# DLR-RM/AugmentedAutoencoder

Hardware: AMD Instinct MI355X
Metric: crops/sec (encode+codebook-NN), 128x128x3 vs 92232x128 codebook, 1/8 GPU (higher is better)
Workload: dtype f32; 1 GPU; configs[1]: single object per GPU, batch=256 uint8 128x128x3 crops, HIP 4-conv encoder -> 128-d + cosine-NN vs 92232x128 fp32 codebook, top-1; batch_per_gpu=256, codebook_rows=92232, latent=128, parallelism=single GPU

## Files before the change

augmentedautoencoder_amd/csrc/kernels/conv_winograd_f32.h:

```cpp
#pragma once
#include <type_traits>

#include "multi_launch.h"

namespace aae {

struct ConvWinoArgs {
    const float* x;
    const float* U;
    const float* bias;
    const float* bn_scale;
    const float* bn_shift;
    float* out;
    int B, H, W, Cin, Cout, Ho, Wo;
    int eh, ew;
    int mode;
    int relu;
    int blocks_x, blocks_y;
    int regions;
    int xcd_cols;
#ifdef AAE_WINO_STAMPS
    long long* stamps;
#endif
};
#ifdef AAE_WINO_STAMPS
constexpr int kWinoStampSlots = 64;
#define AAE_WINO_STAMP(a, slot) do { if ((threadIdx.x & 63) == 0) (a).stamps[((size_t)blockIdx.x * 8 + (threadIdx.x >> 6)) * aae::kWinoStampSlots + (slot)] = aae::clock_ticks(); } while (0)
#else
#define AAE_WINO_STAMP(a, slot) do {} while (0)
#endif
inline unsigned wino_grid_blocks(int regions, int nbn, int xcd_cols) {
    if (xcd_cols <= 0) return (unsigned)regions * (unsigned)nbn;
    const int region_groups = 8 / (nbn / xcd_cols);
    return 8u * (unsigned)xcd_cols * (unsigned)((regions + region_groups - 1) / region_groups);
}
inline bool wino_xcd_cols_valid(int nbn, int xcd_cols) {
    return xcd_cols >= 1 && nbn % xcd_cols == 0 && (nbn / xcd_cols) <= 8 && 8 % (nbn / xcd_cols) == 0;
}

template <int GEOM>
struct WinoGeom;
template <>
struct WinoGeom<0> {
    static constexpr int kImages = 1, kRows = 18, kCols = 18, kRowPitch = 10, kParityPitch = 180, kImagePitch = 2 * 180, kPlane = 2 * 180 + 1;
    static constexpr int kFrameRows = 18, kFrameCols = 18;
    __host__ __device__ static constexpr int image_offset(int) { return 0; }
    __host__ __device__ static constexpr int frame_row(int) { return 0; }
    __host__ __device__ static constexpr int frame_col(int) { return 0; }
};
template <>
struct WinoGeom<1> {
    static constexpr int kImages = 4, kRows = 10, kCols = 10, kRowPitch = 10, kParityPitch = 190, kPlane = 2 * 190 + 1;
    static constexpr int kFrameRows = 19, kFrameCols = 20;
    __host__ __device__ static constexpr int image_offset(int i) { return 90 * (i >> 1) + 5 * (i & 1); }
    __host__ __device__ static constexpr int frame_row(int i) { return 9 * (i >> 1); }
    __host__ __device__ static constexpr int frame_col(int i) { return 10 * (i & 1); }
};
template <>
struct WinoGeom<2> {
    static constexpr int kImages = 4, kRows = 10, kCols = 10, kRowPitch = 6, kParityPitch = 60, kImagePitch = 128, kPlane = 4 * 128 + 1;
    static constexpr int kFrameRows = 10, kFrameCols = 10;
    __host__ __device__ static constexpr int image_offset(int i) { return i * kImagePitch; }
};
template <int GEOM>
constexpr int wino_plane_units() { return WinoGeom<GEOM>::kPlane; }
template <int GEOM>
constexpr int wino_stage_units() { return 8 * wino_plane_units<GEOM>(); }
template <int GEOM>
constexpr int wino_smem_bytes() { return 2 * wino_stage_units<GEOM>() * 16; }
template <int GEOM>
__host__ __device__ constexpr void wino_tile(int mh, int t, int& ti, int& ty, int& tx) {
    const int c = t >> 2, odd = (c ^ (c >> 1) ^ (c >> 2)) & 1;
    if (GEOM == 0) { ti = 0; ty = 4 * mh + (c >> 1); tx = 4 * odd + (t & 3); }
    else if (GEOM == 1) { ti = 2 * mh + odd; ty = c >> 1; tx = t & 3; }
    else { ti = 2 * mh + (t >> 4); ty = (t >> 2) & 3; tx = t & 3; }
}
template <int GEOM>
constexpr bool wino_geom_conflict_free() {
    using G = WinoGeom<GEOM>;
    for (int mh = 0; mh < 2; ++mh)
        for (int set = 0; set < 2; ++set) {
            unsigned seen = 0;
            for (int t = 0; t < 32; ++t) {
                const int c = t >> 2;
                if (((c ^ (c >> 1) ^ (c >> 2)) & 1) != set) continue;
                int ti = 0, ty = 0, tx = 0;
                wino_tile<GEOM>(mh, t, ti, ty, tx);
                seen |= 1u << ((G::image_offset(ti) + 2 * ty * G::kRowPitch + tx) & 15);
            }
            if (seen != 0xffffu) return false;
        }
    unsigned quads = 0;
    for (int cq = 0; cq < 8; ++cq) quads |= 1u << ((cq * G::kPlane) & 15);
    return __builtin_popcount(quads) == 8;
}
static_assert(wino_geom_conflict_free<0>() && wino_geom_conflict_free<1>(), "stage-buffer layouts: patch reads and fill stores free of bank conflicts");

struct ConvWinoLayerArgs {
    ConvWinoArgs c;
    const float* U4[4];
};
struct ConvWinoObject {
    const float* x;
    float* out;
    const float* U4[4];
    const float* bias;
    const float* bn_scale;
    const float* bn_shift;
    int B, pad_;
};
struct ConvWinoMultiArgs {
    ConvWinoArgs c;
    MultiRange range;
    ConvWinoObject obj[kMultiMax];
};
template <int GEOM, int STAGE_CH = 16>
constexpr int wino_layer_stage_bytes() { return 2 * (STAGE_CH / 4) * wino_plane_units<GEOM>() * 16; }
template <int GEOM, int STAGE_CH = 16>
constexpr int wino_layer_smem_bytes() { return wino_layer_stage_bytes<GEOM, STAGE_CH>() + 4 * 64 * 64 * 4; }
static_assert(wino_layer_smem_bytes<0, 32>() <= 160 * 1024 && wino_layer_smem_bytes<1, 32>() <= 160 * 1024 && wino_layer_smem_bytes<2, 16>() <= 160 * 1024, "LDS of a compute unit");
inline int wino_layer_geom_tag(int geom, bool static_halo) { return geom == 0 ? 0 : (static_halo ? 1 : 2); }
inline bool wino_layer_static_halo(int geom, int blocks_x, int blocks_y, bool option) { return option && (geom != 0 || (blocks_x == 1 && blocks_y == 1)); }
inline int wino_layer_stage_channels(int geom, int Cin, bool stage32, bool static_halo = true) {
    return stage32 && (geom == 0 || static_halo) && Cin % 32 == 0 ? 32 : 16;
}


#ifndef AAE_WINO_DECLARATIONS_ONLY

#if defined(__HIP_DEVICE_COMPILE__)
__device__ __forceinline__ f32x2 wino_pk_add(f32x2 a, f32x2 b) {
    f32x2 r;
    asm("v_pk_add_f32 %0, %1, %2" : "=v"(r) : "v"(a), "v"(b));
    return r;
}
__device__ __forceinline__ f32x2 wino_pk_sub(f32x2 a, f32x2 b) {
    f32x2 r;
    asm("v_pk_add_f32 %0, %1, %2 neg_lo:[0,1] neg_hi:[0,1]" : "=v"(r) : "v"(a), "v"(b));
    return r;
}
#else
__host__ __device__ inline f32x2 wino_pk_add(f32x2 a, f32x2 b) { return a + b; }
__host__ __device__ inline f32x2 wino_pk_sub(f32x2 a, f32x2 b) { return a - b; }
#endif
#if defined(__HIP_DEVICE_COMPILE__)
__device__ __forceinline__ f32x4 wino_fma4(float s, f32x4 a, f32x4 b) {
    const f32x2 ss = {s, s};
    f32x2 lo, hi;
    asm("v_pk_fma_f32 %0, %1, %2, %3" : "=v"(lo) : "v"(ss), "v"(a.lo), "v"(b.lo));
    asm("v_pk_fma_f32 %0, %1, %2, %3" : "=v"(hi) : "v"(ss), "v"(a.hi), "v"(b.hi));
    return f32x4{lo.x, lo.y, hi.x, hi.y};
}
#else
__host__ __device__ inline f32x4 wino_fma4(float s, f32x4 a, f32x4 b) {
    f32x4 r;
    for (int e = 0; e < 4; ++e) r[e] = fmaf(s, a[e], b[e]);
    return r;
}
#endif
__device__ __forceinline__ f32x4 wino_add4(f32x4 a, f32x4 b) {
    const f32x2 lo = wino_pk_add(a.lo, b.lo), hi = wino_pk_add(a.hi, b.hi);
    return f32x4{lo.x, lo.y, hi.x, hi.y};
}
__device__ __forceinline__ f32x4 wino_sub4(f32x4 a, f32x4 b) {
    const f32x2 lo = wino_pk_sub(a.lo, b.lo), hi = wino_pk_sub(a.hi, b.hi);
    return f32x4{lo.x, lo.y, hi.x, hi.y};
}
#if defined(__HIP_DEVICE_COMPILE__)
__device__ __forceinline__ float wino_add1(float a, float b) {
    float r;
    asm("v_add_f32 %0, %1, %2" : "=v"(r) : "v"(a), "v"(b));
    return r;
}
__device__ __forceinline__ float wino_sub1(float a, float b) {
    float r;
    asm("v_sub_f32 %0, %1, %2" : "=v"(r) : "v"(a), "v"(b));
    return r;
}
__device__ __forceinline__ float wino_nadd1(float a, float b) {
    float r;
    asm("v_sub_f32 %0, -%1, %2" : "=v"(r) : "v"(a), "v"(b));
    return r;
}
#else
__host__ __device__ inline float wino_add1(float a, float b) { return a + b; }
__host__ __device__ inline float wino_sub1(float a, float b) { return a - b; }
__host__ __device__ inline float wino_nadd1(float a, float b) { return -a - b; }
#endif
template <int N, int M>
__device__ __forceinline__ void wino_acc_fence(f32x16 (&c)[M]) {
#if defined(__HIP_DEVICE_COMPILE__)
    static_assert((N == 3 || N == 6 || N == 8) && N <= M, "PB or 2 PB accumulator tiles");
    if constexpr (N == 8)
        asm volatile("s_nop 15\n\ts_nop 3" : "+v"(c[0]), "+v"(c[1]), "+v"(c[2]), "+v"(c[3]), "+v"(c[4]), "+v"(c[5]), "+v"(c[6]), "+v"(c[7]));
    else if constexpr (N == 6)
        asm volatile("s_nop 15\n\ts_nop 3" : "+v"(c[0]), "+v"(c[1]), "+v"(c[2]), "+v"(c[3]), "+v"(c[4]), "+v"(c[5]));
    else
        asm volatile("s_nop 15\n\ts_nop 3" : "+v"(c[0]), "+v"(c[1]), "+v"(c[2]));
#else
    (void)c;
#endif
}

struct WinoBlock {
    int nb, region, img0, wy0, wx0;
    bool live;
};
__device__ __forceinline__ void wino_block_index(int block, int nbn, int regions, int xcd_cols, WinoBlock& w) {
    if (xcd_cols > 0) {
        const int col_groups = nbn / xcd_cols, region_groups = 8 / col_groups, chunk = (regions + region_groups - 1) / region_groups;
        const int xcd = block & 7, within = block >> 3, k = within / xcd_cols;
        w.nb = (xcd % col_groups) * xcd_cols + within % xcd_cols;
        w.region = (xcd / col_groups) * chunk + k;
        w.live = k < chunk && w.region < regions;
    } else {
        w.nb = block % nbn;
        w.region = block / nbn;
        w.live = w.region < regions;
    }
}
template <int GEOM>
__device__ __forceinline__ void wino_block_geometry(int local, int blocks_x, int blocks_y, WinoBlock& w) {
    if (GEOM == 0) {
        int rest = local;
        const int bx = rest % blocks_x;
        rest /= blocks_x;
        const int by = rest % blocks_y;
        w.img0 = rest / blocks_y;
        w.wy0 = 16 * by - 1;
        w.wx0 = 16 * bx - 1;
    } else {
        w.img0 = 4 * local;
        w.wy0 = w.wx0 = -1;
    }
}
template <int GEOM>
__device__ __forceinline__ WinoBlock wino_block(int block, int nbn, int blocks_x, int blocks_y, int regions, int xcd_cols) {
    WinoBlock w;
    wino_block_index(block, nbn, regions, xcd_cols, w);
    wino_block_geometry<GEOM>(w.region, blocks_x, blocks_y, w);
    return w;
}


template <int GEOM, int STAGE_CH, int NT, bool STATIC = false>
struct WinoFillPlan {
    using G = WinoGeom<GEOM>;
    static constexpr int kQuads = STAGE_CH / 4, kParts = STAGE_CH / 16;
    static constexpr int kDataRows = G::kRows - 2, kDataCols = G::kCols - 2;
    static constexpr int kStageQuads = G::kImages * (STATIC ? kDataRows * kDataCols : G::kRows * G::kCols) * kQuads;
    static constexpr int kPer = ((kStageQuads + NT - 1) / NT + kParts - 1) / kParts;
    static_assert(!STATIC || kStageQuads % (NT * kParts) == 0, "static halo: every thread has the same number of slots");
    static_assert(STATIC || GEOM != 1, "the mosaic's shared zero row needs the static halo");
    uint32_t goff[kParts * kPer];
    int lslot[kParts * kPer];
    __host__ __device__ static constexpr bool wave_stores(int wave, int i) { return STATIC || wave * 64 + NT * i < kStageQuads; }
    static constexpr int kSpareColumn = (G::kCols + 1) / 2;
    static_assert(STATIC || (kSpareColumn < G::kRowPitch && 64 / kQuads <= 2 * G::kRows), "spare units of the stage buffer");
    static_assert(NT % kQuads == 0, "a pixel's quads in one slot round");
    static constexpr int kHaloRows = G::kFrameRows - (G::kFrameRows / (kDataRows + 1)) * kDataRows;
    static constexpr int kHaloCols = G::kFrameCols - (G::kFrameCols / (kDataCols + 2)) * kDataCols;
    static constexpr int kHalo = kHaloRows * G::kFrameCols + (G::kFrameRows - kHaloRows) * kHaloCols;
    static_assert(!STATIC || kHalo + G::kImages * kDataRows * kDataCols == G::kFrameRows * G::kFrameCols, "halo + data = the frame");
};
constexpr uint32_t kWinoOutside = 0x80000000u;
template <int GEOM>
__host__ __device__ constexpr int wino_frame_unit(int fy, int fx) { return (fx & 1) * WinoGeom<GEOM>::kParityPitch + fy * WinoGeom<GEOM>::kRowPitch + (fx >> 1); }
template <int GEOM, int QUADS>
__host__ __device__ constexpr void wino_fill_pixel(int p, int& fy, int& fx) {
    using G = WinoGeom<GEOM>;
    constexpr int DR = G::kRows - 2, DC = G::kCols - 2;
    int wi = p / (DR * DC), dy = p % (DR * DC) / DC, dx = p % DC;
    if (QUADS == 4 && GEOM == 0) {
        const int q = p >> 1;
        wi = 0; dy = q / (DC / 2); dx = (q % (DC / 2)) + (p & 1) * (DC / 2);
    } else if (QUADS == 4) {
        const int q = p >> 1, r = q / DC;
        wi = r >> 2; dy = (r & 1) + 2 * (p & 1) + 4 * ((r >> 1) & 1); dx = q % DC;
    }
    fy = G::frame_row(wi) + 1 + dy;
    fx = G::frame_col(wi) + 1 + dx;
}
template <int GEOM, int QUADS>
constexpr bool wino_fill_order_valid() {
    using G = WinoGeom<GEOM>;
    constexpr int DR = G::kRows - 2, DC = G::kCols - 2, N = G::kImages * DR * DC;
    bool seen[G::kFrameRows * G::kFrameCols] = {};
    for (int p = 0; p < N; ++p) {
        int fy = 0, fx = 0;
        wino_fill_pixel<GEOM, QUADS>(p, fy, fx);
        if (seen[fy * G::kFrameCols + fx]) return false;
        seen[fy * G::kFrameCols + fx] = true;
    }
    for (int p = 0; p < N; p += 8 / QUADS) {
        unsigned banks = 0;
        for (int l = 0; l < 8; ++l) {
            int fy = 0, fx = 0;
            wino_fill_pixel<GEOM, QUADS>(p + l / QUADS, fy, fx);
            banks |= 1u << ((wino_frame_unit<GEOM>(fy, fx) + (l % QUADS) * G::kPlane) & 7);
        }
        if (banks != 0xffu) return false;
    }
    return true;
}
static_assert(wino_fill_order_valid<0, 8>() && wino_fill_order_valid<0, 4>() && wino_fill_order_valid<1, 8>() && wino_fill_order_valid<1, 4>(),
              "static-halo fill order: every data position once, store groups free of bank conflicts");

template <int GEOM, int STAGE_CH, int NT, bool STATIC>
__device__ __forceinline__ void wino_fill_plan(const ConvWinoArgs& a, const WinoBlock& wb, WinoFillPlan<GEOM, STAGE_CH, NT, STATIC>& f) {
    using G = WinoGeom<GEOM>;
    using F = WinoFillPlan<GEOM, STAGE_CH, NT, STATIC>;
    constexpr int kPlane = wino_plane_units<GEOM>();
    const int cq_per_pixel = a.Cin / 4;
    if constexpr (STATIC) {
        const int cq = (int)threadIdx.x % F::kQuads;
#pragma unroll
        for (int i = 0; i < F::kParts * F::kPer; ++i) {
            const int p = ((int)threadIdx.x + NT * i) / F::kQuads, wi = p / (F::kDataRows * F::kDataCols), b = wb.img0 + wi;
            int fy, fx;
            wino_fill_pixel<GEOM, F::kQuads>(p, fy, fx);
            const int uu = fy - G::frame_row(wi) - 1, vv = fx - G::frame_col(wi) - 1;
            f.goff[i] = b < a.B ? (uint32_t)(((((size_t)b * a.H + 2 * uu) * a.W + 2 * vv) * cq_per_pixel + cq) * 16) : kWinoOutside;
            f.lslot[i] = cq * kPlane + wino_frame_unit<GEOM>(fy, fx);
        }
    } else {
        constexpr int kStep = NT / F::kQuads, kWindow = G::kRows * G::kCols;
        constexpr int kStepI = kStep / kWindow, kStepY = kStep % kWindow / G::kCols, kStepX = kStep % G::kCols;
        const int pixel0 = (int)threadIdx.x / F::kQuads, cq = (int)threadIdx.x % F::kQuads;
        int wi = pixel0 / kWindow, wy = pixel0 % kWindow / G::kCols, wx = pixel0 % G::kCols;
#pragma unroll
        for (int i = 0; i < F::kParts * F::kPer; ++i) {
            const int idx = (int)threadIdx.x + NT * i;
            f.goff[i] = kWinoOutside;
            if (idx < F::kStageQuads) {
                const int uu = wb.wy0 + wy, vv = wb.wx0 + wx, b = wb.img0 + wi;
                if (uu >= 0 && uu < a.Ho && vv >= 0 && vv < a.Wo && b < a.B)
                    f.goff[i] = (uint32_t)(((((size_t)b * a.H + 2 * uu) * a.W + 2 * vv) * cq_per_pixel + cq) * 16);
                f.lslot[i] = cq * kPlane + wi * G::kImagePitch + (wx & 1) * G::kParityPitch + wy * G::kRowPitch + (wx >> 1);
            } else {
                const int d = (idx - F::kStageQuads) & 63, row = d / F::kQuads;
                f.lslot[i] = cq * kPlane + (row / G::kRows) * G::kParityPitch + (row % G::kRows) * G::kRowPitch + F::kSpareColumn;
            }
            wx += kStepX;
            wy += kStepY + (wx >= G::kCols ? 1 : 0);
            wx -= wx >= G::kCols ? G::kCols : 0;
            wi += kStepI + (wy >= G::kRows ? 1 : 0);
            wy -= wy >= G::kRows ? G::kRows : 0;
        }
    }
}
template <int GEOM, int STAGE_CH, int NT>
__device__ __forceinline__ void wino_zero_halo(f32x4* lds) {
    using G = WinoGeom<GEOM>;
    using F = WinoFillPlan<GEOM, STAGE_CH, NT, true>;
    constexpr int kStage = F::kQuads * wino_plane_units<GEOM>(), kTotal = 2 * F::kQuads * F::kHalo;
    constexpr int kRowPart = F::kHaloRows * G::kFrameCols, kRowStep = (G::kFrameRows - 1) / (F::kHaloRows - 1);
#pragma unroll
    for (int i = 0; i < (kTotal + NT - 1) / NT; ++i) {
        const int idx = (int)threadIdx.x + NT * i;
        if (idx < kTotal) {
            const int hq = idx % (F::kQuads * F::kHalo), buf = idx / (F::kQuads * F::kHalo), cq = hq % F::kQuads, hp = hq / F::kQuads;
            int fy, fx;
            if (hp < kRowPart) {
                fy = (hp / G::kFrameCols) * kRowStep;
                fx = hp % G::kFrameCols;
            } else {
                const int k = hp - kRowPart, r = k / F::kHaloCols, c = k % F::kHaloCols;
                fy = 1 + r + r / F::kDataRows;
                fx = (c >> 1) * (F::kDataCols + 2) + (c & 1) * (F::kDataCols + 1);
            }
            lds[buf * kStage + cq * wino_plane_units<GEOM>() + wino_frame_unit<GEOM>(fy, fx)] = f32x4{0.f, 0.f, 0.f, 0.f};
        }
    }
}

template <int TA, int TB>
__device__ __forceinline__ void wino_first_fragments(const ConvWinoArgs& a, const float* U, const WinoBlock& wb, f32x4 (&u)[8]) {
    constexpr int PB = TB + 1, NP = (TA + 1) * PB;
    const int tid = threadIdx.x, lane = tid & 63, wave = wave_uniform(tid >> 6);
    const int nh = (wave >> 1) & 1, ph = wave >> 2, m = lane & 31, h = lane >> 5, n32 = wb.nb * 2 + nh, KG = a.Cin / 8;
    const buffer_rsrc urs = make_buffer(U, (uint32_t)((size_t)NP * a.Cin * a.Cout * 4));
    const uint32_t ulane = (uint32_t)(((size_t)n32 * KG * NP + (size_t)ph * 2 * PB) * 64 + h * 32 + m) * 16u;
    const bool two_rows = TA == 3 || ph == 0;
#pragma unroll
    for (int p = 0; p < 2 * PB; ++p) u[p] = buffer_load4_s(urs, ulane + (p % PB) * 1024u, two_rows ? (p / PB) * PB * 1024u : (p / PB) * (NP * 1024u));
}
template <int GEOM, int STAGE_CH, int NT, bool STATIC>
__device__ __forceinline__ void wino_first_stage(const ConvWinoArgs& a, int eh, int ew, const WinoFillPlan<GEOM, STAGE_CH, NT, STATIC>& fill, f32x4* lds) {
    using F = WinoFillPlan<GEOM, STAGE_CH, NT, STATIC>;
    const int wave = wave_uniform((int)threadIdx.x >> 6);
    const buffer_rsrc xrs = make_buffer(a.x, (uint32_t)((size_t)a.B * a.H * a.W * a.Cin * 4));
    const uint32_t parity_off = (uint32_t)(((size_t)eh * a.W + ew) * a.Cin * 4);
    f32x4 stg[F::kParts * F::kPer];
#pragma unroll
    for (int i = 0; i < F::kParts * F::kPer; ++i) stg[i] = buffer_load4_s(xrs, fill.goff[i], parity_off);
    if constexpr (STATIC) wino_zero_halo<GEOM, STAGE_CH, NT>(lds);
#pragma unroll
    for (int i = 0; i < F::kParts * F::kPer; ++i)
        if (F::wave_stores(wave, i)) lds[fill.lslot[i]] = stg[i];
    __syncthreads();
}

template <int TA, int TB, bool SWAP, int GEOM, int STAGE_CH, bool ACCUMULATE, bool WIDE, int CHAIN = 0, int NTA = 3, int NTB = 3, bool STATIC = false>
__device__ __forceinline__ void wino_phase_body(const ConvWinoArgs& a, const float* U, int eh, int ew, const WinoBlock& wb, f32x4* lds, float* xch_all,
                                                const WinoFillPlan<GEOM, STAGE_CH, WIDE ? 256 : 512, STATIC>& fill, int& buf0, f32x4 (&uin)[8],
                                                const float* Un, int neh, int new_, f32x4 (&uout)[8]) {
    using G = WinoGeom<GEOM>;
    using F = WinoFillPlan<GEOM, STAGE_CH, WIDE ? 256 : 512, STATIC>;
    constexpr int PB = TB + 1;
    constexpr int kQuads = STAGE_CH / 4, kGroups = STAGE_CH / 8;
    constexpr int kPlane = wino_plane_units<GEOM>(), kStage = kQuads * kPlane;
    constexpr int kParity = G::kParityPitch;
    constexpr int kParts = F::kParts, kPer = F::kPer;
    constexpr int NH = WIDE ? 2 : 1;
    constexpr int kOffA = TA == 2 ? 1 : 0, kOffB = TB == 2 ? 1 : 0;
    static_assert(!STATIC || (CHAIN & 1), "the static halo is written in front of the chained form's first stage (wino_first_stage)");
    static_assert(CHAIN == 0 || !WIDE, "the chained form passes one wave's weight fragments between the components");
    const int tid = threadIdx.x, lane = tid & 63, wave = wave_uniform(tid >> 6);
    const int mh = wave & 1, nh = WIDE ? 0 : (wave >> 1) & 1, ph = WIDE ? wave >> 1 : wave >> 2, m = lane & 31, h = lane >> 5;
    int li, lty, ltx;
    wino_tile<GEOM>(mh, m, li, lty, ltx);
    const int n32 = wb.nb * 2 + nh, KG = a.Cin / 8, nst = a.Cin / STAGE_CH;
    constexpr int NP = (TA + 1) * PB;
    constexpr int kPhaseNo = TA == 3 && TB == 3 ? 0 : (TA == 3 && !SWAP ? 1 : (TA == 3 ? 2 : 3));
    (void)kPhaseNo;
    AAE_WINO_STAMP(a, 4 * kPhaseNo + 0);
    const buffer_rsrc xrs = make_buffer(a.x, (uint32_t)((size_t)a.B * a.H * a.W * a.Cin * 4));
    const buffer_rsrc urs = make_buffer(U, (uint32_t)((size_t)NP * a.Cin * a.Cout * 4));
    const uint32_t ulane = (uint32_t)(((size_t)n32 * KG * NP + (size_t)ph * 2 * PB) * 64 + h * 32 + m) * 16u;
    const bool two_rows = TA == 3 || ph == 0;
    const uint32_t parity_off = (uint32_t)(((size_t)eh * a.W + ew) * a.Cin * 4);
    const uint32_t next_parity_off = (uint32_t)(((size_t)neh * a.W + new_) * a.Cin * 4);

    f32x16 acc[NH][2 * PB];

    f32x4 stg[kPer];
    auto stage_load = [&](uint32_t soff, int part) {
#pragma unroll
        for (int i = 0; i < kPer; ++i) stg[i] = buffer_load4_s(xrs, fill.goff[part * kPer + i], soff);
    };
    auto stage_store = [&](int buf, int part) {
#pragma unroll
        for (int i = 0; i < kPer; ++i)
            if (F::wave_stores(wave, part * kPer + i)) lds[buf * kStage + fill.lslot[part * kPer + i]] = stg[i];
    };
    auto fA = [](int pos) { return SWAP ? (pos & 1) * kParity + (pos >> 1) : pos * G::kRowPitch; };
    auto fB = [](int pos) { return SWAP ? pos * G::kRowPitch : (pos & 1) * kParity + (pos >> 1); };
    const int lane_base = G::image_offset(li) + 2 * lty * G::kRowPitch + ltx;
    const int posA0 = (TA == 3 ? (ph == 0 ? 0 : 2) : (ph == 0 ? 0 : 1)) + kOffA;
    const int posA1 = (ph == 0 ? 1 : 3) + kOffA;
    const int posA2 = (TA == 3 ? (ph == 0 ? 2 : 1) : (ph == 0 ? 1 : 2)) + kOffA;
    const int offA0 = fA(posA0), offA1 = fA(posA1), offA2 = fA(posA2);
    const float sg = ph == 0 ? 1.f : -1.f;

    const uint32_t half_stride = (uint32_t)KG * NP * 1024u;
    f32x4 u[NH][2 * PB];
    if (CHAIN & 1) {
#pragma unroll
        for (int p = 0; p < 2 * PB; ++p) u[0][p] = uin[p];
    } else {
#pragma unroll
        for (int n2 = 0; n2 < NH; ++n2)
#pragma unroll
            for (int p = 0; p < 2 * PB; ++p)
                u[n2][p] = buffer_load4_s(urs, ulane + (p % PB) * 1024u, (two_rows ? (p / PB) * PB * 1024u : (p / PB) * (NP * 1024u)) + n2 * half_stride);
#pragma unroll
        for (int part = 0; part < kParts; ++part) {
            stage_load(parity_off, part);
            stage_store(buf0, part);
        }
        __syncthreads();
    }
    AAE_WINO_STAMP(a, 4 * kPhaseNo + 1);

    auto read_unit = [&](const f32x4* plane, int i, f32x4 (&raw)[2 * PB]) {
#pragma unroll
        for (int s2 = 0; s2 < PB; ++s2) {
            const int ob = fB(s2 + kOffB);
            if (i == 0) raw[s2] = plane[offA0 + ob];
            else if (TA == 3) raw[s2] = plane[offA1 + ob];
            if (i == 0) raw[PB + s2] = plane[offA2 + ob];
        }
    };
    auto step_a = [&](int i, const f32x4 (&raw)[2 * PB], f32x4 (&w)[PB]) {
#pragma unroll
        for (int s2 = 0; s2 < PB; ++s2) {
            if (i == 0) w[s2] = wino_sub4(raw[s2], raw[PB + s2]);
            else if (TA == 3) w[s2] = wino_fma4(sg, raw[s2], raw[PB + s2]);
            else w[s2] = raw[PB + s2];
        }
    };
    auto step_b = [&](f32x4 (&w)[PB]) {
        if (TB == 3) {
            const f32x4 e0 = w[0], e1 = w[1], e2 = w[2], e3 = w[PB - 1];
            w[0] = wino_sub4(e0, e2);
            w[1] = wino_add4(e1, e2);
            w[2] = wino_sub4(e2, e1);
            w[PB - 1] = wino_sub4(e1, e3);
        } else {
            const f32x4 e0 = w[0], e1 = w[1], e2 = w[2];
            w[0] = wino_sub4(e0, e1);
            w[2] = wino_sub4(e1, e2);
        }
    };
    auto run = [&](auto rows_tag) {
        constexpr int ROWS = decltype(rows_tag)::value, NU = kGroups * ROWS, kPartUnits = NU / kParts;
        static_assert(NU % 2 == 0 && NU % kParts == 0, "units per stage");
        constexpr int kStoreBack = kPartUnits >= 4 ? 2 : 1;
        const bool early = ph == 1 && kStoreBack == 2;
        f32x4 raw[2 * PB], v[PB];
        read_unit(lds + buf0 * kStage + h * kPlane + lane_base, 0, raw);
        auto stage_body = [&](int st, auto first_tag) {
            constexpr bool FIRST = decltype(first_tag)::value;
            const int buf = (buf0 + st) & 1;
            const bool more = st + 1 < nst;
            const bool filling = more || (CHAIN & 2);
            const uint32_t fill_off = more ? parity_off + (uint32_t)(st + 1) * kQuads * 16 : next_parity_off;
#ifdef AAE_WINO_STAMPS
            if (kPhaseNo == 0 && st < 8) AAE_WINO_STAMP(a, 20 + st);
#endif
            const f32x4* stage = lds + buf * kStage + h * kPlane + lane_base;
            const f32x4* next_stage = lds + (buf ^ 1) * kStage + h * kPlane + lane_base;
#pragma unroll
            for (int t = 0; t < NU; ++t) {
                const int i = t % ROWS, slot = t & 1;
#ifdef AAE_WINO_STAMPS
                if (kPhaseNo == 0 && (st == 2 || st == 3) && t < 4) AAE_WINO_STAMP(a, 28 + 6 * (st - 2) + t);
#endif
                step_a(i, raw, v);
                step_b(v);
                if ((!FIRST || t > 0) && (more || t + 1 < NU)) {
                    const int tn = (t + 1) % NU, gn = (st + (t + 1) / NU) * kGroups + tn / ROWS;
                    const uint32_t un = (uint32_t)gn * (NP * 1024u) + (tn % ROWS) * PB * 1024u;
#pragma unroll
                    for (int n2 = 0; n2 < NH; ++n2)
#pragma unroll
                        for (int j = 0; j < PB; ++j) u[n2][(slot ^ 1) * PB + j] = buffer_load4_s(urs, ulane + j * 1024u, un + n2 * half_stride);
                }
                if (filling && t % kPartUnits == 0) stage_load(fill_off, t / kPartUnits);
                if (filling && t % kPartUnits == kPartUnits - kStoreBack) stage_store(buf ^ 1, t / kPartUnits);
                if (t + 1 < NU) read_unit(stage + 2 * ((t + 1) / ROWS) * kPlane, (t + 1) % ROWS, raw);
                if (filling && (t == NU - 1 ? !early : (t == NU - 2 && early))) {
#ifdef AAE_WINO_STAMPS
                    if (kPhaseNo == 0 && (st == 2 || st == 3)) AAE_WINO_STAMP(a, 28 + 6 * (st - 2) + 4);
#endif
                    __syncthreads();
#ifdef AAE_WINO_STAMPS
                    if (kPhaseNo == 0 && (st == 2 || st == 3)) AAE_WINO_STAMP(a, 28 + 6 * (st - 2) + 5);
#endif
                }
                if (t == NU - 1 && more) read_unit(next_stage, 0, raw);
                sched_fence();
#pragma unroll
                for (int q = 0; q < 4; ++q)
#pragma unroll
                    for (int j = 0; j < PB; ++j)
#pragma unroll
                        for (int n2 = 0; n2 < NH; ++n2) {
                            f32x16& c = acc[n2][(ROWS == 2 ? i * PB : 0) + j];
                            if (FIRST && t < ROWS && q == 0) c = mfma_32x32x2(v[j][q], u[n2][slot * PB + j][q], f32x16{});
                            else c = mfma_32x32x2(v[j][q], u[n2][slot * PB + j][q], c);
                        }
                sched_fence();
            }
        };
        stage_body(0, std::true_type());
        for (int st = 1; st < nst; ++st) stage_body(st, std::false_type());
    };
    if (TA == 3 || ph == 0) run(std::integral_constant<int, 2>());
    else run(std::integral_constant<int, 1>());
    if (STAGE_CH == 32 && CHAIN == 0) __syncthreads();
    AAE_WINO_STAMP(a, 4 * kPhaseNo + 2);
    if (CHAIN & 2) {
        wino_first_fragments<NTA, NTB>(a, Un, wb, uout);
    }
    buf0 = (buf0 + nst) & 1;
#pragma unroll
    for (int n2 = 0; n2 < NH; ++n2) {
        if constexpr (TA == 2) {
            if (ph == 1) wino_acc_fence<PB>(acc[n2]);
            else wino_acc_fence<2 * PB>(acc[n2]);
        } else {
            wino_acc_fence<2 * PB>(acc[n2]);
        }
    }

    auto drain = [&](auto ph_tag) {
        constexpr int PH = decltype(ph_tag)::value;
        auto partial = [&](int n2, int r, float (&y)[4]) {
            constexpr bool kNoQ0 = PH == 1 && TA == 2;
            float q0[PB], q1[PB];
#pragma unroll
            for (int j = 0; j < PB; ++j) {
                const float mA = acc[n2][j][r], mB = kNoQ0 ? 0.f : acc[n2][PB + j][r];
                if (PH == 0) { q0[j] = wino_add1(mA, mB); q1[j] = mB; }
                else if (TA == 3) { q0[j] = mA; q1[j] = wino_nadd1(mA, mB); }
                else { q0[j] = 0.f; q1[j] = -mA; }
            }
            float t[4];
            if (TB == 3) {
                t[0] = kNoQ0 ? 0.f : wino_add1(wino_add1(q0[0], q0[1]), q0[2]);
                t[1] = kNoQ0 ? 0.f : wino_sub1(wino_sub1(q0[1], q0[2]), q0[3]);
                t[2] = wino_add1(wino_add1(q1[0], q1[1]), q1[2]);
                t[3] = wino_sub1(wino_sub1(q1[1], q1[2]), q1[3]);
            } else {
                t[0] = kNoQ0 ? 0.f : wino_add1(q0[0], q0[1]);
                t[1] = kNoQ0 ? 0.f : wino_sub1(q0[1], q0[2]);
                t[2] = wino_add1(q1[0], q1[1]);
                t[3] = wino_sub1(q1[1], q1[2]);
            }
            y[0] = t[0];
            y[1] = SWAP ? t[2] : t[1];
            y[2] = SWAP ? t[1] : t[2];
            y[3] = t[3];
        };
        f32x4 yv[NH][16];
#pragma unroll
        for (int n2 = 0; n2 < NH; ++n2)
#pragma unroll
            for (int r = 0; r < 16; ++r) {
                float y[4];
                partial(n2, r, y);
                yv[n2][r] = f32x4{y[0], y[1], y[2], y[3]};
            }
#ifdef AAE_WINO_STAMPS
        AAE_WINO_STAMP(a, 48 + 4 * kPhaseNo + 0);
#endif
#pragma unroll
        for (int round = 0; round < 2; ++round) {
            const int par = PH == round ? 0 : 1;
#pragma unroll
            for (int n2 = 0; n2 < NH; ++n2) {
                f32x4* xq = reinterpret_cast<f32x4*>(xch_all) + (size_t)(mh + 2 * (nh + n2)) * 16 * 64 + lane;
                if (ACCUMULATE || round == 1) {
                    f32x4 old[8];
#pragma unroll
                    for (int e = 0; e < 8; ++e) old[e] = xq[(2 * e + par) * 64];
#pragma unroll
                    for (int e = 0; e < 8; ++e) xq[(2 * e + par) * 64] = old[e] + yv[n2][2 * e + par];
                } else {
#pragma unroll
                    for (int e = 0; e < 8; ++e) xq[(2 * e + par) * 64] = yv[n2][2 * e + par];
                }
            }
#ifdef AAE_WINO_STAMPS
            asm volatile("s_waitcnt lgkmcnt(0)" ::: "memory");
            AAE_WINO_STAMP(a, 48 + 4 * kPhaseNo + 1 + 2 * round);
#endif
            if (round == 0 || !(CHAIN & 2) || nst < 2) __syncthreads();
#ifdef AAE_WINO_STAMPS
            if (round == 0) AAE_WINO_STAMP(a, 48 + 4 * kPhaseNo + 2);
#endif
        }
    };
    if (ph == 0) drain(std::integral_constant<int, 0>());
    else drain(std::integral_constant<int, 1>());
    AAE_WINO_STAMP(a, 4 * kPhaseNo + 3);
}

template <int GEOM, int NT>
__device__ __forceinline__ void wino_store_block(const ConvWinoArgs& a, int mode, const WinoBlock& wb, const float* xall) {
    const int tid = threadIdx.x;
    const int n4 = wb.nb * 64 + (tid & 15) * 4;
    f32x4 bs = {0.f, 0.f, 0.f, 0.f}, sc = {1.f, 1.f, 1.f, 1.f}, sh = {0.f, 0.f, 0.f, 0.f};
    if (mode >= 2) {
        bs = *reinterpret_cast<const f32x4*>(a.bias + n4);
        if (a.bn_scale) {
            sc = *reinterpret_cast<const f32x4*>(a.bn_scale + n4);
            sh = *reinterpret_cast<const f32x4*>(a.bn_shift + n4);
        }
    }
#pragma unroll
    for (int round = 0; round < 1024 / NT; ++round) {
        const int idx = tid + NT * round, cq = idx & 15, t = idx >> 4;
        const int tmh = t >> 5, mt = t & 31, tnh = cq >> 3;
        const int r = (mt & 3) + 4 * (mt >> 3), hh = (mt >> 2) & 1;
        const f32x4* src = reinterpret_cast<const f32x4*>(xall) + (size_t)(tmh + 2 * tnh) * 16 * 64 + r * 64 + 32 * hh + (cq & 7) * 4;
        const f32x4 c0 = src[0], c1 = src[1], c2 = src[2], c3 = src[3];
        int ti, ty, tx;
        wino_tile<GEOM>(tmh, mt, ti, ty, tx);
        const int b = wb.img0 + ti;
        if (b >= a.B) continue;
        const int oy = (GEOM == 0 ? wb.wy0 + 1 : 0) + 2 * ty, ox = (GEOM == 0 ? wb.wx0 + 1 : 0) + 2 * tx;
        float* o = a.out + (((size_t)b * a.Ho + oy) * a.Wo + ox) * a.Cout + wb.nb * 64 + cq * 4;
        float* optr[4] = {o, o + a.Cout, o + (size_t)a.Wo * a.Cout, o + (size_t)a.Wo * a.Cout + a.Cout};
        f32x4 val[4];
#pragma unroll
        for (int k = 0; k < 4; ++k) val[k] = f32x4{c0[k], c1[k], c2[k], c3[k]};
        if (mode == 1 || mode == 2) {
#pragma unroll
            for (int k = 0; k < 4; ++k) val[k] += *reinterpret_cast<const f32x4*>(optr[k]);
        }
        if (mode >= 2) {
#pragma unroll
            for (int k = 0; k < 4; ++k) {
                val[k] += bs;
                if (a.relu) {
#pragma unroll
                    for (int e = 0; e < 4; ++e) val[k][e] = fmaxf(val[k][e], 0.f);
                }
                if (a.bn_scale) val[k] = val[k] * sc + sh;
            }
        }
#pragma unroll
        for (int k = 0; k < 4; ++k) *reinterpret_cast<f32x4*>(optr[k]) = val[k];
    }
}

#ifdef AAE_EXPERIMENTS
template <int TA, int TB, bool SWAP, int GEOM>
__global__ __launch_bounds__(512) void conv_wino_phase_kernel(ConvWinoArgs a) {
    AAE_DYN_SMEM(smem_raw);
    const WinoBlock wb = wino_block<GEOM>(blockIdx.x, a.Cout / 64, a.blocks_x, a.blocks_y, a.regions, a.xcd_cols);
    if (!wb.live) return;
    WinoFillPlan<GEOM, 32, 512> fill;
    wino_fill_plan(a, wb, fill);
    int buf0 = 0;
    f32x4 unused[8];
    wino_phase_body<TA, TB, SWAP, GEOM, 32, false, false>(a, a.U, a.eh, a.ew, wb, reinterpret_cast<f32x4*>(smem_raw), reinterpret_cast<float*>(smem_raw), fill, buf0, unused,
                                                          nullptr, 0, 0, unused);
    wino_store_block<GEOM, 512>(a, a.mode, wb, reinterpret_cast<const float*>(smem_raw));
}
#endif

template <int GEOM, bool WIDE, int STAGE_CH, bool STATIC>
__device__ __forceinline__ void wino_layer_block(const ConvWinoArgs& a, const float* const (&U4)[4], const WinoBlock& wb, unsigned char* smem_raw) {
    constexpr int SC = STAGE_CH;
    static_assert(SC == 16 || (SC == 32 && !WIDE), "stage size");
    static_assert(!STATIC || !WIDE, "the static halo belongs to the chained form");
    f32x4* lds = reinterpret_cast<f32x4*>(smem_raw);
    float* xch = reinterpret_cast<float*>(smem_raw + wino_layer_stage_bytes<GEOM, SC>());
    WinoFillPlan<GEOM, SC, WIDE ? 256 : 512, STATIC> fill;
    int buf0 = 0;
    f32x4 ua[8], ub[8];
    if (!WIDE) wino_first_fragments<3, 3>(a, U4[3], wb, ua);
    wino_fill_plan(a, wb, fill);
    if constexpr (WIDE) {
        wino_phase_body<3, 3, false, GEOM, SC, false, WIDE>(a, U4[3], 1, 1, wb, lds, xch, fill, buf0, ua, nullptr, 0, 0, ub);
        wino_phase_body<3, 2, false, GEOM, SC, true, WIDE>(a, U4[2], 1, 0, wb, lds, xch, fill, buf0, ua, nullptr, 0, 0, ub);
        wino_phase_body<3, 2, true, GEOM, SC, true, WIDE>(a, U4[1], 0, 1, wb, lds, xch, fill, buf0, ua, nullptr, 0, 0, ub);
        wino_phase_body<2, 2, false, GEOM, SC, true, WIDE>(a, U4[0], 0, 0, wb, lds, xch, fill, buf0, ua, nullptr, 0, 0, ub);
    } else {
        constexpr bool W = WIDE;
        if (!W) wino_first_stage(a, 1, 1, fill, lds);
        wino_phase_body<3, 3, false, GEOM, SC, false, W, W ? 0 : 3, 3, 2, STATIC>(a, U4[3], 1, 1, wb, lds, xch, fill, buf0, ua, U4[2], 1, 0, ub);
        wino_phase_body<3, 2, false, GEOM, SC, true, W, W ? 0 : 3, 3, 2, STATIC>(a, U4[2], 1, 0, wb, lds, xch, fill, buf0, ub, U4[1], 0, 1, ua);
        wino_phase_body<3, 2, true, GEOM, SC, true, W, W ? 0 : 3, 2, 2, STATIC>(a, U4[1], 0, 1, wb, lds, xch, fill, buf0, ua, U4[0], 0, 0, ub);
        wino_phase_body<2, 2, false, GEOM, SC, true, W, W ? 0 : 1, 3, 3, STATIC>(a, U4[0], 0, 0, wb, lds, xch, fill, buf0, ub, nullptr, 0, 0, ua);
    }
    wino_store_block<GEOM, WIDE ? 256 : 512>(a, 3, wb, xch);
}

template <int GEOM, bool WIDE, int STAGE_CH = 16, bool STATIC = false>
__global__ __launch_bounds__(WIDE ? 256 : 512) void conv_wino_layer_kernel(ConvWinoLayerArgs p) {
    AAE_DYN_SMEM(smem_raw);
    const ConvWinoArgs& a = p.c;
    const WinoBlock wb = wino_block<GEOM>(blockIdx.x, a.Cout / 64, a.blocks_x, a.blocks_y, a.regions, a.xcd_cols);
    if (!wb.live) return;
    wino_layer_block<GEOM, WIDE, STAGE_CH, STATIC>(a, p.U4, wb, smem_raw);
#ifdef AAE_WINO_STAMPS
    asm volatile("s_waitcnt vmcnt(0)" ::: "memory");
    AAE_WINO_STAMP(a, 16);
    if (threadIdx.x == 0) a.stamps[((size_t)blockIdx.x * 8) * kWinoStampSlots + 17] = (long long)(__builtin_amdgcn_s_getreg(20 | (0 << 6) | (3 << 11)) & 15);
#endif
}

template <int GEOM, int STAGE_CH = 16, bool STATIC = false>
__global__ __launch_bounds__(512) void conv_wino_layer_multi_kernel(ConvWinoMultiArgs p) {
    AAE_DYN_SMEM(smem_raw);
    WinoBlock wb;
    wino_block_index(blockIdx.x, p.c.Cout / 64, p.c.regions, p.c.xcd_cols, wb);
    if (!wb.live) return;
    const int o = multi_find(p.range, wb.region);
    wino_block_geometry<GEOM>(wb.region - p.range.first[o], p.c.blocks_x, p.c.blocks_y, wb);
    ConvWinoArgs a = p.c;
    const ConvWinoObject& ob = p.obj[o];
    a.x = ob.x; a.out = ob.out; a.bias = ob.bias; a.bn_scale = ob.bn_scale; a.bn_shift = ob.bn_shift; a.B = ob.B;
    const float* U4[4] = {ob.U4[0], ob.U4[1], ob.U4[2], ob.U4[3]};
    wino_layer_block<GEOM, false, STAGE_CH, STATIC>(a, U4, wb, smem_raw);
}

#endif

}
```

Measured before the change: 58170 crops/s.

## Split static-halo fill across four waves and drain Winograd outputs in pairs

For the chained 32-channel static-halo Winograd layer, the input staging fill is handed to the four ph==0 waves, each holding one base offset plus compile-time strides, in place of per-slot offset tables spread over all eight waves. The output drain is reworked to pack element pairs with packed-float adds and write the exchange buffer as float4 pairs, with a matching pair-aware store routine and a permuted row-to-tile mapping. The aim is to cut fill-plan register use, the number of LDS transactions and the scalar drain instructions. In exchange, half the waves sit idle during fills, so the remaining waves carry a heavier load and more latency lands on the critical path.

Result: no change. 58070 crops/s (-0.2%).

```diff
diff --git a/augmentedautoencoder_amd/csrc/kernels/conv_winograd_f32.h b/augmentedautoencoder_amd/csrc/kernels/conv_winograd_f32.h
--- a/augmentedautoencoder_amd/csrc/kernels/conv_winograd_f32.h
+++ b/augmentedautoencoder_amd/csrc/kernels/conv_winograd_f32.h
@@ -75,6 +75,17 @@
     else if (GEOM == 1) { ti = 2 * mh + odd; ty = c >> 1; tx = t & 3; }
     else { ti = 2 * mh + (t >> 4); ty = (t >> 2) & 3; tx = t & 3; }
 }
+template <int STAGE_CH, bool WIDE>
+constexpr bool wino_drain_pairs() {
+#ifdef AAE_WINO_SCALAR_DRAIN
+    return false;
+#else
+    return STAGE_CH == 32 && !WIDE;
+#endif
+}
+template <bool PAIRS>
+__host__ __device__ constexpr int wino_row_tile(int m) { return PAIRS ? (m & ~3) | ((m & 1) << 1) | ((m >> 1) & 1) : m; }
+
 template <int GEOM>
 constexpr bool wino_geom_conflict_free() {
     using G = WinoGeom<GEOM>;
@@ -139,9 +150,15 @@
     asm("v_pk_add_f32 %0, %1, %2 neg_lo:[0,1] neg_hi:[0,1]" : "=v"(r) : "v"(a), "v"(b));
     return r;
 }
+__device__ __forceinline__ f32x2 wino_pk_nadd(f32x2 a, f32x2 b) {
+    f32x2 r;
+    asm("v_pk_add_f32 %0, %1, %2 neg_lo:[1,1] neg_hi:[1,1]" : "=v"(r) : "v"(a), "v"(b));
+    return r;
+}
 #else
 __host__ __device__ inline f32x2 wino_pk_add(f32x2 a, f32x2 b) { return a + b; }
 __host__ __device__ inline f32x2 wino_pk_sub(f32x2 a, f32x2 b) { return a - b; }
+__host__ __device__ inline f32x2 wino_pk_nadd(f32x2 a, f32x2 b) { return -a - b; }
 #endif
 #if defined(__HIP_DEVICE_COMPILE__)
 __device__ __forceinline__ f32x4 wino_fma4(float s, f32x4 a, f32x4 b) {
@@ -306,6 +323,84 @@
 static_assert(wino_fill_order_valid<0, 8>() && wino_fill_order_valid<0, 4>() && wino_fill_order_valid<1, 8>() && wino_fill_order_valid<1, 4>(),
               "static-halo fill order: every data position once, store groups free of bank conflicts");
 
+template <int GEOM, int STAGE_CH, bool WIDE, bool STATIC>
+constexpr bool wino_fill_split() {
+#ifdef AAE_WINO_FILL_ALL_WAVES
+    return false;
+#else
+    return STATIC && STAGE_CH == 32 && !WIDE;
+#endif
+}
+template <int GEOM>
+struct WinoFillSplit {
+    using G = WinoGeom<GEOM>;
+    using P = WinoFillPlan<GEOM, 32, 256, true>;
+    static constexpr int kQuads = P::kQuads, kParts = P::kParts, kPer = P::kPer, kSlots = kParts * kPer, kPixelStep = 256 / kQuads;
+    static_assert(kPer * 4 <= 16, "at most 16 staging registers live at a time");
+    uint32_t goff;
+    int lslot;
+    int images;
+    struct Step { int wi, uu, vv, units; };
+    __host__ __device__ static constexpr Step step_from(int p0, int i) {
+        constexpr int kImagePixels = P::kDataRows * P::kDataCols;
+        const int p = p0 + kPixelStep * i, wi0 = p0 / kImagePixels, wi = p / kImagePixels;
+        int fy0 = 0, fx0 = 0, fy = 0, fx = 0;
+        wino_fill_pixel<GEOM, kQuads>(p0, fy0, fx0);
+        wino_fill_pixel<GEOM, kQuads>(p, fy, fx);
+        return Step{wi - wi0, (fy - G::frame_row(wi)) - (fy0 - G::frame_row(wi0)), (fx - G::frame_col(wi)) - (fx0 - G::frame_col(wi0)),
+                    wino_frame_unit<GEOM>(fy, fx) - wino_frame_unit<GEOM>(fy0, fx0)};
+    }
+    __host__ __device__ static constexpr Step step(int i) { return step_from(0, i); }
+    static constexpr bool regular() {
+        for (int p0 = 0; p0 < kPixelStep; ++p0) {
+            if (p0 >= P::kDataRows * P::kDataCols) return false;
+            for (int i = 0; i < kSlots; ++i) {
+                const Step s = step_from(p0, i), s0 = step(i);
+                if (s.wi != s0.wi || s.uu != s0.uu || s.vv != s0.vv || s.units != s0.units) return false;
+            }
+        }
+        return true;
+    }
+    __host__ __device__ static uint32_t source_step(const ConvWinoArgs& a, int i) {
+        const Step s = step(i);
+        return (uint32_t)(((s.wi * a.H + 2 * s.uu) * a.W + 2 * s.vv) * a.Cin * 4);
+    }
+};
+static_assert(WinoFillSplit<0>::regular() && WinoFillSplit<1>::regular(), "the four-wave fill of the static halo: one offset pair per thread");
+template <int GEOM, int STAGE_CH, bool WIDE, bool STATIC>
+using WinoLayerFill = std::conditional_t<wino_fill_split<GEOM, STAGE_CH, WIDE, STATIC>(), WinoFillSplit<GEOM>, WinoFillPlan<GEOM, STAGE_CH, WIDE ? 256 : 512, STATIC>>;
+
+template <int GEOM>
+__device__ __forceinline__ void wino_fill_plan(const ConvWinoArgs& a, const WinoBlock& wb, WinoFillSplit<GEOM>& f) {
+    using G = WinoGeom<GEOM>;
+    using F = WinoFillSplit<GEOM>;
+    const int t = (int)threadIdx.x & 255, cq = t % F::kQuads, p = t / F::kQuads;
+    int fy, fx;
+    wino_fill_pixel<GEOM, F::kQuads>(p, fy, fx);
+    const int uu = fy - G::frame_row(0) - 1, vv = fx - G::frame_col(0) - 1;
+    f.goff = (uint32_t)(((((size_t)wb.img0 * a.H + 2 * uu) * a.W + 2 * vv) * (a.Cin / 4) + cq) * 16);
+    f.lslot = cq * wino_plane_units<GEOM>() + wino_frame_unit<GEOM>(fy, fx);
+    f.images = a.B - wb.img0;
+}
+template <int GEOM>
+__device__ __forceinline__ void wino_split_load(const ConvWinoArgs& a, const WinoFillSplit<GEOM>& f, uint32_t soff, int part, f32x4 (&stg)[WinoFillSplit<GEOM>::kPer]) {
+    using F = WinoFillSplit<GEOM>;
+    const uint32_t bytes = (uint32_t)((size_t)a.B * a.H * a.W * a.Cin * 4);
+#pragma unroll
+    for (int i = 0; i < F::kPer; ++i) {
+        const int k = part * F::kPer + i;
+        const bool inside = WinoGeom<GEOM>::kImages == 1 || F::step(k).wi < f.images;
+        stg[i] = buffer_load4_s(make_buffer(a.x, inside ? bytes : 0u), f.goff, soff + F::source_step(a, k));
+    }
+}
+template <int GEOM>
+__device__ __forceinline__ void wino_split_store(const WinoFillSplit<GEOM>& f, f32x4* stage_buffer, int part, const f32x4 (&stg)[WinoFillSplit<GEOM>::kPer]) {
+    using F = WinoFillSplit<GEOM>;
+    f32x4* slot0 = stage_buffer + f.lslot;
+#pragma unroll
+    for (int i = 0; i < F::kPer; ++i) slot0[F::step(part * F::kPer + i).units] = stg[i];
+}
+
 template <int GEOM, int STAGE_CH, int NT, bool STATIC>
 __device__ __forceinline__ void wino_fill_plan(const ConvWinoArgs& a, const WinoBlock& wb, WinoFillPlan<GEOM, STAGE_CH, NT, STATIC>& f) {
     using G = WinoGeom<GEOM>;
@@ -400,13 +495,31 @@
         if (F::wave_stores(wave, i)) lds[fill.lslot[i]] = stg[i];
     __syncthreads();
 }
+template <int GEOM>
+__device__ __forceinline__ void wino_first_stage(const ConvWinoArgs& a, int eh, int ew, const WinoFillSplit<GEOM>& fill, f32x4* lds) {
+    using F = WinoFillSplit<GEOM>;
+    const int wave = wave_uniform((int)threadIdx.x >> 6);
+    const uint32_t parity_off = (uint32_t)(((size_t)eh * a.W + ew) * a.Cin * 4);
+    f32x4 stg[F::kParts][F::kPer];
+    if (wave < 4) {
+#pragma unroll
+        for (int part = 0; part < F::kParts; ++part) wino_split_load(a, fill, parity_off, part, stg[part]);
+    }
+    wino_zero_halo<GEOM, 32, 512>(lds);
+    if (wave < 4) {
+#pragma unroll
+        for (int part = 0; part < F::kParts; ++part) wino_split_store(fill, lds, part, stg[part]);
+    }
+    __syncthreads();
+}
 
 template <int TA, int TB, bool SWAP, int GEOM, int STAGE_CH, bool ACCUMULATE, bool WIDE, int CHAIN = 0, int NTA = 3, int NTB = 3, bool STATIC = false>
 __device__ __forceinline__ void wino_phase_body(const ConvWinoArgs& a, const float* U, int eh, int ew, const WinoBlock& wb, f32x4* lds, float* xch_all,
-                                                const WinoFillPlan<GEOM, STAGE_CH, WIDE ? 256 : 512, STATIC>& fill, int& buf0, f32x4 (&uin)[8],
+                                                const WinoLayerFill<GEOM, STAGE_CH, WIDE, STATIC>& fill, int& buf0, f32x4 (&uin)[8],
                                                 const float* Un, int neh, int new_, f32x4 (&uout)[8]) {
     using G = WinoGeom<GEOM>;
-    using F = WinoFillPlan<GEOM, STAGE_CH, WIDE ? 256 : 512, STATIC>;
+    using F = WinoLayerFill<GEOM, STAGE_CH, WIDE, STATIC>;
+    constexpr bool kSplitFill = wino_fill_split<GEOM, STAGE_CH, WIDE, STATIC>();
     constexpr int PB = TB + 1;
     constexpr int kQuads = STAGE_CH / 4, kGroups = STAGE_CH / 8;
     constexpr int kPlane = wino_plane_units<GEOM>(), kStage = kQuads * kPlane;
@@ -418,8 +531,9 @@
     static_assert(CHAIN == 0 || !WIDE, "the chained form passes one wave's weight fragments between the components");
     const int tid = threadIdx.x, lane = tid & 63, wave = wave_uniform(tid >> 6);
     const int mh = wave & 1, nh = WIDE ? 0 : (wave >> 1) & 1, ph = WIDE ? wave >> 1 : wave >> 2, m = lane & 31, h = lane >> 5;
+    constexpr bool kPairs = wino_drain_pairs<STAGE_CH, WIDE>() && CHAIN != 0;
     int li, lty, ltx;
-    wino_tile<GEOM>(mh, m, li, lty, ltx);
+    wino_tile<GEOM>(mh, wino_row_tile<kPairs>(m), li, lty, ltx);
     const int n32 = wb.nb * 2 + nh, KG = a.Cin / 8, nst = a.Cin / STAGE_CH;
     constexpr int NP = (TA + 1) * PB;
     constexpr int kPhaseNo = TA == 3 && TB == 3 ? 0 : (TA == 3 && !SWAP ? 1 : (TA == 3 ? 2 : 3));
@@ -436,13 +550,21 @@
 
     f32x4 stg[kPer];
     auto stage_load = [&](uint32_t soff, int part) {
-#pragma unroll
-        for (int i = 0; i < kPer; ++i) stg[i] = buffer_load4_s(xrs, fill.goff[part * kPer + i], soff);
+        if constexpr (kSplitFill) {
+            if (ph == 0) wino_split_load(a, fill, soff, part, stg);
+        } else {
+#pragma unroll
+            for (int i = 0; i < kPer; ++i) stg[i] = buffer_load4_s(xrs, fill.goff[part * kPer + i], soff);
+        }
     };
     auto stage_store = [&](int buf, int part) {
-#pragma unroll
-        for (int i = 0; i < kPer; ++i)
-            if (F::wave_stores(wave, part * kPer + i)) lds[buf * kStage + fill.lslot[part * kPer + i]] = stg[i];
+        if constexpr (kSplitFill) {
+            if (ph == 0) wino_split_store(fill, lds + buf * kStage, part, stg);
+        } else {
+#pragma unroll
+            for (int i = 0; i < kPer; ++i)
+                if (F::wave_stores(wave, part * kPer + i)) lds[buf * kStage + fill.lslot[part * kPer + i]] = stg[i];
+        }
     };
     auto fA = [](int pos) { return SWAP ? (pos & 1) * kParity + (pos >> 1) : pos * G::kRowPitch; };
     auto fB = [](int pos) { return SWAP ? pos * G::kRowPitch : (pos & 1) * kParity + (pos >> 1); };
@@ -653,8 +775,85 @@
 #endif
         }
     };
-    if (ph == 0) drain(std::integral_constant<int, 0>());
-    else drain(std::integral_constant<int, 1>());
+    auto drain_pairs = [&](auto ph_tag) {
+        constexpr int PH = decltype(ph_tag)::value;
+        constexpr bool kNoQ0 = PH == 1 && TA == 2;
+        f32x4 yv[16];
+#pragma unroll
+        for (int e = 0; e < 8; ++e) {
+            f32x2 mA[PB], mB[PB], t[4];
+#pragma unroll
+            for (int j = 0; j < PB; ++j) {
+                mA[j] = f32x2{acc[0][j][2 * e], acc[0][j][2 * e + 1]};
+                if (!kNoQ0) mB[j] = f32x2{acc[0][PB + j][2 * e], acc[0][PB + j][2 * e + 1]};
+            }
+            if constexpr (kNoQ0) {
+                t[0] = t[1] = f32x2{0.f, 0.f};
+                if (TB == 3) {
+                    t[2] = wino_pk_sub(wino_pk_nadd(mA[0], mA[1]), mA[2]);
+                    t[3] = wino_pk_add(wino_pk_sub(mA[2], mA[1]), mA[PB - 1]);
+                } else {
+                    t[2] = wino_pk_nadd(mA[0], mA[1]);
+                    t[3] = wino_pk_sub(mA[2], mA[1]);
+                }
+            } else {
+                f32x2 q0[PB], q1[PB];
+#pragma unroll
+                for (int j = 0; j < PB; ++j) {
+                    if (PH == 0) { q0[j] = wino_pk_add(mA[j], mB[j]); q1[j] = mB[j]; }
+                    else { q0[j] = mA[j]; q1[j] = wino_pk_nadd(mA[j], mB[j]); }
+                }
+                if (TB == 3) {
+                    t[0] = wino_pk_add(wino_pk_add(q0[0], q0[1]), q0[2]);
+                    t[1] = wino_pk_sub(wino_pk_sub(q0[1], q0[2]), q0[PB - 1]);
+                    t[2] = wino_pk_add(wino_pk_add(q1[0], q1[1]), q1[2]);
+                    t[3] = wino_pk_sub(wino_pk_sub(q1[1], q1[2]), q1[PB - 1]);
+                } else {
+                    t[0] = wino_pk_add(q0[0], q0[1]);
+                    t[1] = wino_pk_sub(q0[1], q0[2]);
+                    t[2] = wino_pk_add(q1[0], q1[1]);
+                    t[3] = wino_pk_sub(q1[1], q1[2]);
+                }
+            }
+            const f32x2 y1 = SWAP ? t[2] : t[1], y2 = SWAP ? t[1] : t[2];
+            yv[2 * e] = f32x4{t[0].x, t[0].y, y1.x, y1.y};
+            yv[2 * e + 1] = f32x4{y2.x, y2.y, t[3].x, t[3].y};
+        }
+#ifdef AAE_WINO_STAMPS
+        AAE_WINO_STAMP(a, 48 + 4 * kPhaseNo + 0);
+#endif
+        f32x4* xq = reinterpret_cast<f32x4*>(xch_all) + (size_t)(mh + 2 * nh) * 16 * 64 + lane;
+#pragma unroll
+        for (int round = 0; round < 2; ++round) {
+            const int par = PH == round ? 0 : 1;
+            auto slot = [&](int k) { return 2 * (2 * (k >> 1) + par) + (k & 1); };
+            if (ACCUMULATE || round == 1) {
+                f32x4 old[8];
+#pragma unroll
+                for (int k = 0; k < 8; ++k) old[k] = xq[slot(k) * 64];
+#pragma unroll
+                for (int k = 0; k < 8; ++k) xq[slot(k) * 64] = old[k] + yv[slot(k)];
+            } else {
+#pragma unroll
+                for (int k = 0; k < 8; ++k) xq[slot(k) * 64] = yv[slot(k)];
+            }
+#ifdef AAE_WINO_STAMPS
+            asm volatile("s_waitcnt lgkmcnt(0)" ::: "memory");
+            AAE_WINO_STAMP(a, 48 + 4 * kPhaseNo + 1 + 2 * round);
+#endif
+            if (round == 0 || !(CHAIN & 2) || nst < 2) __syncthreads();
+#ifdef AAE_WINO_STAMPS
+            if (round == 0) AAE_WINO_STAMP(a, 48 + 4 * kPhaseNo + 2);
+#endif
+        }
+    };
+    if constexpr (kPairs) {
+        if (ph == 0) drain_pairs(std::integral_constant<int, 0>());
+        else drain_pairs(std::integral_constant<int, 1>());
+    } else {
+        if (ph == 0) drain(std::integral_constant<int, 0>());
+        else drain(std::integral_constant<int, 1>());
+    }
     AAE_WINO_STAMP(a, 4 * kPhaseNo + 3);
 }
 
@@ -707,6 +906,58 @@
     }
 }
 
+template <int GEOM>
+__device__ __forceinline__ void wino_store_block_pairs(const ConvWinoArgs& a, int mode, const WinoBlock& wb, const float* xall) {
+    const int tid = threadIdx.x, cq = tid & 15, tp = tid >> 4;
+    const int n4 = wb.nb * 64 + cq * 4;
+    f32x4 bs = {0.f, 0.f, 0.f, 0.f}, sc = {1.f, 1.f, 1.f, 1.f}, sh = {0.f, 0.f, 0.f, 0.f};
+    if (mode >= 2) {
+        bs = *reinterpret_cast<const f32x4*>(a.bias + n4);
+        if (a.bn_scale) {
+            sc = *reinterpret_cast<const f32x4*>(a.bn_scale + n4);
+            sh = *reinterpret_cast<const f32x4*>(a.bn_shift + n4);
+        }
+    }
+    const int tmh = tp >> 4, e = tp & 7, hh = (tp >> 3) & 1, tnh = cq >> 3;
+    const f32x4* src = reinterpret_cast<const f32x4*>(xall) + (size_t)(tmh + 2 * tnh) * 16 * 64 + 2 * e * 64 + 32 * hh + (cq & 7) * 4;
+    f32x4 c[2][4];
+#pragma unroll
+    for (int half = 0; half < 2; ++half)
+#pragma unroll
+        for (int j = 0; j < 4; ++j) c[half][j] = src[half * 64 + j];
+#pragma unroll
+    for (int d = 0; d < 2; ++d) {
+        const int r = 2 * e + d, row = (r & 3) + 8 * (r >> 2) + 4 * hh;
+        int ti, ty, tx;
+        wino_tile<GEOM>(tmh, wino_row_tile<true>(row), ti, ty, tx);
+        const int b = wb.img0 + ti;
+        if (b >= a.B) break;
+        const int oy = (GEOM == 0 ? wb.wy0 + 1 : 0) + 2 * ty, ox = (GEOM == 0 ? wb.wx0 + 1 : 0) + 2 * tx;
+        float* o = a.out + (((size_t)b * a.Ho + oy) * a.Wo + ox) * a.Cout + n4;
+        float* optr[4] = {o, o + a.Cout, o + (size_t)a.Wo * a.Cout, o + (size_t)a.Wo * a.Cout + a.Cout};
+        f32x4 val[4];
+#pragma unroll
+        for (int k = 0; k < 4; ++k) val[k] = f32x4{c[k >> 1][0][2 * (k & 1) + d], c[k >> 1][1][2 * (k & 1) + d], c[k >> 1][2][2 * (k & 1) + d], c[k >> 1][3][2 * (k & 1) + d]};
+        if (mode == 1 || mode == 2) {
+#pragma unroll
+            for (int k = 0; k < 4; ++k) val[k] += *reinterpret_cast<const f32x4*>(optr[k]);
+        }
+        if (mode >= 2) {
+#pragma unroll
+            for (int k = 0; k < 4; ++k) {
+                val[k] += bs;
+                if (a.relu) {
+#pragma unroll
+                    for (int el = 0; el < 4; ++el) val[k][el] = fmaxf(val[k][el], 0.f);
+                }
+                if (a.bn_scale) val[k] = val[k] * sc + sh;
+            }
+        }
+#pragma unroll
+        for (int k = 0; k < 4; ++k) *reinterpret_cast<f32x4*>(optr[k]) = val[k];
+    }
+}
+
 #ifdef AAE_EXPERIMENTS
 template <int TA, int TB, bool SWAP, int GEOM>
 __global__ __launch_bounds__(512) void conv_wino_phase_kernel(ConvWinoArgs a) {
@@ -730,7 +981,7 @@
     static_assert(!STATIC || !WIDE, "the static halo belongs to the chained form");
     f32x4* lds = reinterpret_cast<f32x4*>(smem_raw);
     float* xch = reinterpret_cast<float*>(smem_raw + wino_layer_stage_bytes<GEOM, SC>());
-    WinoFillPlan<GEOM, SC, WIDE ? 256 : 512, STATIC> fill;
+    WinoLayerFill<GEOM, SC, WIDE, STATIC> fill;
     int buf0 = 0;
     f32x4 ua[8], ub[8];
     if (!WIDE) wino_first_fragments<3, 3>(a, U4[3], wb, ua);
@@ -748,7 +999,8 @@
         wino_phase_body<3, 2, true, GEOM, SC, true, W, W ? 0 : 3, 2, 2, STATIC>(a, U4[1], 0, 1, wb, lds, xch, fill, buf0, ua, U4[0], 0, 0, ub);
         wino_phase_body<2, 2, false, GEOM, SC, true, W, W ? 0 : 1, 3, 3, STATIC>(a, U4[0], 0, 0, wb, lds, xch, fill, buf0, ub, nullptr, 0, 0, ua);
     }
-    wino_store_block<GEOM, WIDE ? 256 : 512>(a, 3, wb, xch);
+    if constexpr (wino_drain_pairs<SC, WIDE>()) wino_store_block_pairs<GEOM>(a, 3, wb, xch);
+    else wino_store_block<GEOM, WIDE ? 256 : 512>(a, 3, wb, xch);
 }
 
 template <int GEOM, bool WIDE, int STAGE_CH = 16, bool STATIC = false>
```
